# tesseract-robotics/trajopt

Measured on AMD Instinct MI355X. Metric: SQP iters/s (+ QP solves/s), 7-DOF x 30-wp x 1024-batch glass_upright, higher is better.
Workload: dtype f64; 1 GPU; config 1: glass_upright 7-DOF 30-waypoint, collision cost, batch=1024 random seeds per GPU; n_dof=7, n_steps=30, batch_per_gpu=1024, qp_n=572, qp_m=876, parallelism=seeds sharded, dp1

## Files before the change

trajopt_amd/csrc/tmx_api.cpp:

```cpp
#include <algorithm>
#include <cstddef>
#include <limits>
#include <string>
#include <vector>

#include "tmx_kernels.h"
#include "tmx_wave_kernels.h"
#include "tmx_wave_plan.h"
#include "tmx_row_perm.h"
#include "tmx_upload.h"

#ifdef TMX_HOST_EMU
#include <chrono>
thread_local tmx_emu_idx tmx_emu_threadIdx, tmx_emu_blockIdx, tmx_emu_blockDim, tmx_emu_gridDim;
thread_local double* tmx_emu_smem = nullptr;
double tmx_emu_now_ms()
{
  return std::chrono::duration<double, std::milli>(std::chrono::steady_clock::now().time_since_epoch()).count();
}
#else
#include <rccl/rccl.h>
#endif

#define HIPCHK(call)                                                                                                  \
// ... 1396 lines not shown
    int acc = 0, rows_max = 0, naux_max = 0;
    for (int t = 0; t <= T; ++t)
    {
      pl.pst[t] = acc;
      if (t == T)
        break;
      const int c = L.wp_start[t + 1] - L.wp_start[t];
      for (int u = L.wp_start[t]; u < L.wp_start[t + 1]; ++u)
        pl.epos[L.wp_list[u]] = acc + (u - L.wp_start[t]);
      acc += c + (c & 1);
      rows_max = std::max(rows_max, c);
    }
    for (int r = 0; r < R; ++r)
      naux_max = std::max(naux_max, L.naux[r]);
    pl.setup_fast = (rows_max <= TMX_SETUP_COL && naux_max <= 2 && R <= 2 * TMX_QP_NT) ? 1 : 0;
    pl.polish_fast = 0;
    if (pl.setup_fast && dpart_fits(D, T) && R2 == 0)
    {
      DPart dp;
      dpart_make(T, dp);
      const size_t gn = (size_t)dp.Lmax * D, g_doubles = (size_t)dp.P * gn * dpart_gstride((int)gn);
      pl.polish_fast = polish_fast_doubles(T, D * T, R, NA, acc + TMX_SETUP_COL) <= g_doubles ? 1 : 0;
    }
  }
  pl.smem_small = small_smem_bytes(L, P);
#if TMX_IS_DEVICE
  {
    std::vector<int> plan(TMX_WV_NT * TMX_WV_REC, 0);
    int gmax = 4, aux2 = 0, n3 = 0;
    if (hooks.wave == '1' && P.flavor == 0 && R2 == 0 && pl.coef_far == 0 && !E.qp_dense && !P.st && !P.band && !P.use_time && P.n_fx == 0 &&
        wave_plan_build(D, T, R, L.st.data(), L.naux.data(), plan.data(), &gmax, &aux2, &n3))
    {
      const size_t lds = std::max(pl.smem_small, wave_lds_doubles(D, T, R) * sizeof(double));
      if (lds <= 40 * 1024)
      {
        pl.plan.swap(plan);
        pl.wave_ok = 1;
        pl.wv_gmax = gmax;
        pl.wv_aux2 = aux2;
        pl.smem_wave = lds;
      }
    }
  }
#endif
  pl.smem_qp = qp_smem_bytes(D, T, R, NA, R2, pl.coef_far);
  if (P.tt_chain > 0 || P.tv_chain)
// ... 97 lines not shown
  UP(cp_target, L.cp_target);
  UP(ls_link, L.ls_link);
  UP(ls_center, L.ls_center);
  UP(ls_radius, L.ls_radius);
  UP(ob_center, L.ob_center);
  UP(ob_radius, L.ob_radius);
  UP(ob_axis, L.ob_axis);
  UP(tv_owner, L.tv_owner);
  UP(tv_joint, L.tv_joint);
  UP(tv_first, L.tv_first);
  UP(tv_last, L.tv_last);
  UP(tv_coeff, L.tv_coeff);
  UP(tv_target, L.tv_target);
  UP(tv_up, L.tv_up);
  UP(tv_lo, L.tv_lo);
  UP(tt_owner, L.tt_owner);
  UP(tt_form, L.tt_form);
  UP(tt_slot, L.tt_slot);
  UP(tt_coeff, L.tt_coeff);
  UP(tt_limit, L.tt_limit);
  P.coef_far = pl.coef_far;
  P.setup_fast = pl.setup_fast;
  P.polish_fast = pl.polish_fast;
  P.tt_place = pl.tt_place;
  P.wave_ok = pl.wave_ok;
  P.wv_gmax = pl.wv_gmax;
  P.wv_aux2 = pl.wv_aux2;
  if (!pl.row_perm.empty())
    UP(row_perm, pl.row_perm);
  UP(wp_pst, pl.pst);
  UP(row_epos, pl.epos);
  if (pl.wave_ok)
    UP(wv_plan, pl.plan);
#undef UP
  if (!ctx->dp)
  {
    void* p = nullptr;
    HIPCHK(hipMalloc(&p, sizeof(DevProblem)));
    ctx->dp = static_cast<DevProblem*>(p);
  }
  HIPCHK(hipMemcpy(ctx->dp, &P, sizeof(DevProblem), hipMemcpyHostToDevice));
  return TMX_OK;
}

static tmx_status configure_launch(tmx_ctx* ctx, const DevProblem& P, const Lowered& L, const EngineChoice& E, const Placement& pl, const UploadHooks& hooks)
{
// ... 1465 lines not shown
  if (!ctx || !ctx->have_problem || !ctx->dp)
    return TMX_ERR_INVALID;
  TMX_REFUSE_WHILE_PENDING(ctx);
  HIPCHK(hipSetDevice(ctx->device));
  ctx->hp.dbg_flags = flags;
  HIPCHK(hipMemcpy(reinterpret_cast<char*>(ctx->dp) + offsetof(DevProblem, dbg_flags), &flags, sizeof(int), hipMemcpyHostToDevice));
  return TMX_OK;
}

__attribute__((visibility("default"))) int tmx_debug_setup_fast(tmx_ctx* ctx)
{
  if (!ctx || !ctx->have_problem)
    return -1;
  return ctx->hp.setup_fast;
}

__attribute__((visibility("default"))) int tmx_debug_polish_fast(tmx_ctx* ctx)
{
  if (!ctx || !ctx->have_problem)
    return -1;
  return ctx->hp.polish_fast;
}

__attribute__((visibility("default"))) tmx_status tmx_debug_set_fused(tmx_ctx* ctx, int mode)
{
  if (!ctx || mode < 0 || mode > 2)
    return TMX_ERR_INVALID;
  ctx->mode = mode;
  return TMX_OK;
}

tmx_status tmx_kernel_stats_reset(tmx_ctx* ctx)
{
  if (!ctx)
    return TMX_ERR_INVALID;
  ctx->ms_admm = ctx->ms_convexify = ctx->ms_evaluate = 0.0;
  ctx->launches_admm = 0;
  return TMX_OK;
}
}
```

trajopt_amd/csrc/tmx_kernels.h:

```cpp
#pragma once
#include "tmx_solve.h"
#include "tmx_generic.h"

#define TMX_WORK(smem, Bt) ((Bt)->ws_hbm ? (Bt)->ws_hbm + (size_t)blockIdx.x * (size_t)(Bt)->ws_hbm_stride : (smem))

template <bool HULL>
TMX_DEVFN void prepare_body(const DevProblem* P, const DevBatch* Bt)
{
  TMX_SMEM(smem);
  const int b = blockIdx.x, tid = threadIdx.x, NT = blockDim.x;
  const int NX = P->NX, D = P->D, R = P->R;
  const double* x0 = Bt->x0 + (size_t)b * NX;
  double* x = Bt->x + (size_t)b * NX;
  for (int v = tid; v < NX; v += NT)
  {
    const int j = v % D;
    double y = fmax(P->jl[j] + 1e-6, x0[v]);
    y = fmin(P->ju[j] - 1e-6, x0[v]);
    x[v] = (P->flavor == 1) ? x0[v] : y;
  }
  int* act = Bt->active + (size_t)b * R;
  for (int r = tid; r < R; r += NT)
    act[r] = 0;
  for (int k = tid; k < P->n_cnts; k += NT)
// ... 356 lines not shown
#ifdef TMX_PROFILE
  long long tp0 = TMX_CLK();
  const long long wall0 = wall_clock64();
#endif
  if (P->sqp.max_time < 1e300)
  {
    if (tid == 0)
      sqp_time_limit_check(P, Bt, b);
    TMX_SYNC();
    if (Bt->phase[b] == PHASE_DONE)
      return;
  }
  if (Bt->phase[b] == PHASE_CONVEXIFY)
  {
    convexify_terms(P, x, act, coef, Bt->coef2 + (size_t)b * P->n_link * D, rhs, smem, tid, NT, Bt->rowc + (size_t)b * R, Bt->qdyn + (size_t)b * NX);
#ifdef TMX_PROFILE
    if (tid == 0)
    {
      const long long tnow = TMX_CLK();
      Bt->prof[(size_t)b * 16 + 4] += tnow - tp0;
      tp0 = tnow;
    }
#endif
    QpWs cwd;
    qp_structure(P, act, coef, Bt->coef2 + (size_t)b * P->n_link * D, rhs, x, Bt->trust[b], Bt->merit + (size_t)b * P->n_cnts, Bt->dims + 4 * b,
                 Bt->hashes + 4 * b, nullptr, reinterpret_cast<int*>(smem), tid, NT, Bt->qdyn + (size_t)b * NX, compact_lists_of(cwd, P, Bt, b));
#if TMX_LINK_ROWS
    if (P->flavor == 1)
      sqp2_begin_qp(P, Bt, b, smem, tid, NT);
#endif
  }
  TMX_SYNC();
#ifdef TMX_PROFILE
  if (tid == 0)
    Bt->prof[(size_t)b * 16 + 11] += TMX_CLK() - tp0;
#endif
  qp_solve_block<HBM, BANDK, false>(P, Bt, b, smem, tid, NT, chain_lds);
#ifdef TMX_PROFILE
  tp0 = TMX_CLK();
#endif
  for (int v = tid; v < NX; v += NT)
    xn[v] = xq[v];
  TMX_SYNC();
  evaluate_terms(P, xn, Bt->new_cost_vals + (size_t)b * P->n_costs, Bt->new_cnt_viols + (size_t)b * P->n_cnts, smem, tid, NT);
#if TMX_LINK_ROWS
  if (P->flavor == 1)
    sqp2_update_block(P, Bt, b, smem, tid, NT);
  else
#endif
    sqp_update_block(P, Bt, b, smem, tid, NT);
  TMX_SYNC();
#ifdef TMX_PROFILE
  if (tid == 0)
  {
    Bt->prof[(size_t)b * 16 + 12] += TMX_CLK() - tp0;
    Bt->prof[(size_t)b * 16 + 1] += wall_clock64() - wall0;
  }
#endif
}

TMX_KERNEL_LB2(TMX_QP_NT, TMX_QP_WGS_PER_CU) k_sqp_fused(const DevProblem* P, const DevBatch* Bt, int max_steps)
{
  TMX_SMEM(smem);
  const int b = blockIdx.x, tid = threadIdx.x, NT = blockDim.x;
  for (int step = 0; max_steps == 0 || step < max_steps; ++step)
  {
    if (Bt->phase[b] == PHASE_DONE)
      break;
    if (P->band)
      sqp_step_block<false, true>(P, Bt, b, smem, tid, NT);
    else
      sqp_step_block<false, false>(P, Bt, b, smem, tid, NT);
  }
// ... 297 lines not shown
```

trajopt_amd/csrc/tmx_setup.h:

```cpp
#pragma once
#include "tmx_qp.h"

#if TMX_IS_DEVICE
struct SetupRow
{
  int r, t, na, ao, epos;
  bool on;
  double c[8], sa[2], bba[2], qa[2], Da[2], Eba[2], Er;
};

TMX_DEVFN double ruiz_fast(const QpWs& w, const DevProblem* P, int n_pass, int n, int tid)
{
  constexpr int NT = TMX_QP_NT;
  const int D = w.D, T = w.T, NX = w.NX, R = w.R;
  for (int e = tid; e < T * 8; e += NT)
    w.tp[e] = 0.0;
  for (int e = tid; e < R + T + TMX_SETUP_COL; e += NT)
    w.hr[e] = 0.0;
  SetupRow g[2];
  {
    const int* rperm = P->row_perm;
#pragma unroll
    for (int q = 0; q < 2; ++q)
    {
      SetupRow& s = g[q];
      const int slot = q * NT + tid;
// ... 202 lines not shown
```

trajopt_amd/csrc/tmx_solve.h:

```cpp
#pragma once
#include "tmx_qp.h"
#include "tmx_setup.h"
#include "tmx_polish.h"
#include "tmx_terms.h"

#if TMX_IS_DEVICE
#define TMX_ATOMIC_ADD_U64(ptr, v) atomicAdd((unsigned long long*)(ptr), (unsigned long long)(v))
#else
#define TMX_ATOMIC_ADD_U64(ptr, v) __atomic_fetch_add((unsigned long long*)(ptr), (unsigned long long)(v), __ATOMIC_RELAXED)
#endif

TMX_DEVFN double aux_cost(const DevProblem* P, const double* merit, int r)
{
  if (P->flavor == 1)
  {
    const double cf = (P->slot_kind[r] == SLOT_COLLISION_LVS) ? P->slot_objc[r] : P->slot_scale[r];
    return (P->slot_iscnt[r] ? merit[P->slot_owner[r]] : 1.0) * cf;
  }
  return P->slot_iscnt[r] ? merit[P->slot_owner[r]] : P->slot_objc[r];
}
TMX_DEVFN double primary_q(const DevProblem* P, const double* qdyn, int v)
{
  if (P->flavor == 1)
    return (fabs(qdyn[v]) < 1e-7) ? 0.0 : qdyn[v];
  return P->pq[v];
}

TMX_DEVFN double aux_sign(int naux, int k) { return (naux == 1) ? -1.0 : (k == 0 ? 1.0 : -1.0); }

struct CscOut
{
  long long *P_p, *P_i, *A_p, *A_i;
// ... 53 lines not shown
      {
        const int sgm = side ? t - 1 : t;
        if (sgm < P->tv_first[c] || sgm >= P->tv_last[c])
          continue;
        const double* rec = tv_aff + ((size_t)c * P->T + sgm) * TMX_TV_REC;
        double cf = 0.0;
        if (j == P->D - 1)
          cf = side ? rec[2] : 0.0;
        else if (j == P->tv_joint[c])
          cf = side ? rec[1] : rec[0];
        if (half)
          cf = -cf;
        const double lin = ((2 * rec[3 + half]) * cf) * P->tv_coeff[c];
        if (lin != 0.0)
          qv += lin;
      }
  return qv;
}

template <bool ST = false>
TMX_DEVFN void qp_structure(const DevProblem* P, const int* active, const double* coef, const double* coef2, const double* rhs,
                            const double* xcur, double trust, const double* merit, int* dims, unsigned long long* hashes,
                            const CscOut* out, int* iscratch, int tid, int NT, const double* qdyn = nullptr, QpWs* cw = nullptr,
                            const double* fxH = nullptr, const double* fxg = nullptr, const double* tv_aff = nullptr, const double* tt_aff = nullptr)
{
  (void)coef2;
  (void)fxH;
  (void)fxg;
  (void)tv_aff;
  (void)tt_aff;
  const int D = P->D, T = P->T, NX = P->NX, R = P->R;
  int* colptr = iscratch;
  int* rowref = colptr + P->n_max + 1;
  int* auxref = rowref + R;
  int* lact = auxref + R;
  int* lnaux = lact + R;
  int* ccount = lnaux + R;
  int acc_off = 2 * (P->n_max + 1) + 4 * R;
  acc_off += (acc_off & 1);
  unsigned long long* acc = reinterpret_cast<unsigned long long*>(iscratch + acc_off);
  int* scan = iscratch + acc_off + 16;
  for (int r = tid; r < R; r += NT)
  {
    lact[r] = active[r] ? 1 : 0;
    lnaux[r] = P->slot_naux[r];
  }
  for (int k = tid; k < 8; k += NT)
// ... 85 lines not shown
    ccount[v] = c;
  }
  for (int rq = tid; rq < n_it; rq += NT)
  {
    const int r = ali ? ali[rq] : rq;
    if (lact[r])
      for (int k = 0; k < lnaux[r]; ++k)
        ccount[auxref[r] + k] = 2;
  }
  TMX_SYNC();
  for (int c = tid; c <= n; c += NT)
  {
    int run = 0;
    for (int q = 0; q < c; ++q)
      run += ccount[q];
    colptr[c] = run;
    if (c == n)
    {
      dims[3] = run;
      dims[2] = P->nnzP;
    }
  }
  TMX_SYNC();
  const int nnzA = dims[3];
  unsigned long long hA = 0ULL, wsA = 0ULL;
  const int cp_bytes = n + 1, cp_full = cp_bytes / 8, cp_rem = cp_bytes % 8;
  const int ri_bytes = nnzA, ri_full = ri_bytes / 8, ri_rem = ri_bytes % 8;
  for (int c = tid; c <= n; c += NT)
  {
    const long long val = colptr[c];
    hA += tmx_hash_term(val, (uint64_t)c, 3);
    if (c < cp_full)
      wsA += tmx_hash_term(val, (uint64_t)c, 13);
    else if (c == cp_full && cp_rem > 0)
      wsA += tmx_hash_term((long long)((unsigned long long)val & ((1ULL << (8 * cp_rem)) - 1ULL)), (uint64_t)c, 13);
  }
  for (int v = tid; v < NX; v += NT)
  {
    const int t = v / D, j = v % D;
    int pos = colptr[v];
#if TMX_LINK_ROWS
    int ql = (P->n_link > 0 && t > 0) ? wls[t - 1] : 0;
    const int ql_end = (P->n_link > 0 && t > 0) ? wls[t] : 0;
    auto link_val = [&](int qq) -> double {
      const int rr = wll[qq];
      return (active[rr] && P->slot_c2[rr] >= 0) ? coef2[P->slot_c2[rr] * D + j] : 0.0;
// ... 141 lines not shown
    const int r = ali ? ali[rq] : rq;
    if (active[r])
      for (int k = 0; k < P->slot_naux[r]; ++k)
      {
        const int col = auxref[r] + k;
        int pos = colptr[col];
        for (int e = 0; e < 2; ++e)
        {
          const long long ri = (e == 0) ? rowref[r] : (mg + col);
          hA += tmx_hash_term(ri, (uint64_t)pos, 4);
          if (pos < ri_full)
            wsA += tmx_hash_term(ri, (uint64_t)pos, 14);
          else if (pos == ri_full && ri_rem > 0)
            wsA += tmx_hash_term((long long)((unsigned long long)ri & ((1ULL << (8 * ri_rem)) - 1ULL)), (uint64_t)pos, 14);
          if (out)
          {
            out->A_i[pos] = ri;
            out->A_x[pos] = (e == 0) ? aux_sign(P->slot_naux[r], k) : 1.0;
          }
          ++pos;
        }
      }
  }
  unsigned long long hP = 0ULL, wsP = 0ULL;
  bool p_done = false;
  if constexpr (ST)
    if ((fxH != nullptr && P->n_fx_cost > 0) || (tv_aff != nullptr && P->n_tv > 0) || (tt_aff != nullptr && P->n_tt > 0))
    {
      p_done = true;
      TMX_SYNC();
      int* pcnt = ccount;
      const int T1 = P->T + 1;
      auto fx_val = [&](int t, int i, int j, bool& any) -> double {
        double v = 0.0;
        any = false;
        if (fxH == nullptr)
          return v;
        for (int c = 0; c < P->n_fx; ++c)
          if (fx_is_quad(P->fx_kind[c]) && P->fx_t[c] == t)
          {
            const double h = fxH[(size_t)P->fx_ci[c] * D * D + i * D + j];
            const double coeff = (i == j) ? h / 2 : h;
            if (coeff != 0.0)
            {
              v += (i == j) ? 2.0 * coeff : coeff;
              any = true;
// ... 1098 lines not shown
      w.row_epos[P->wp_list[u]] = acc + (u - P->wp_start[t]);
  }
#if TMX_LINK_ROWS
  w.c2i = P->slot_c2;
#endif
  w.sigma = st.sigma;
  w.alpha = st.alpha;
  w.c = 1.0;
  w.cinv = 1.0;
  TMX_SYNC();
  {
    int* scan = reinterpret_cast<int*>(w.red);
    const int C = (R + NT - 1) / NT;
    const int r0 = tid * C < R ? tid * C : R, r1 = (tid + 1) * C < R ? (tid + 1) * C : R;
    for (int pass = 0; pass < 2; ++pass)
    {
      int cnt = 0;
      for (int r = r0; r < r1; ++r)
        cnt += w.act[r] ? (pass == 0 ? 1 : w.naux[r]) : 0;
      int off = 0;
#if TMX_IS_DEVICE
      if (fast_setup)
      {
        const int lane = tid & 63, wave = tid >> 6;
        const unsigned long long below = (1ull << lane) - 1ull;
        int tot = 0;
        for (int bit = 0; bit < 3; ++bit)
        {
          const unsigned long long mk = __builtin_amdgcn_ballot_w64(((cnt >> bit) & 1) != 0);
          off += __builtin_popcountll(mk & below) << bit;
          tot += __builtin_popcountll(mk) << bit;
        }
        TMX_SYNC();
        if (lane == 0)
          scan[wave] = tot;
        TMX_SYNC();
        for (int u = 0; u < wave; ++u)
          off += scan[u];
      }
      else
#endif
      {
        TMX_SYNC();
        scan[tid] = cnt;
        TMX_SYNC();
        for (int u = 0; u < tid; ++u)
          off += scan[u];
      }
      for (int r = r0; r < r1; ++r)
      {
        if (pass == 0)
          w.row_ref[r] = off;
        else
          w.aux_ref[r] = NX + off;
        off += w.act[r] ? (pass == 0 ? 1 : w.naux[r]) : 0;
      }
    }
    TMX_SYNC();
    rows_compact_build(w, P, scan, tid, NT);
  }
  const int n = dims[0], m = dims[1], mg = m - n;
// ... 1101 lines not shown
                for (int tt = 1; tt < P->T; ++tt)
                {
                  if (g[tt] == 0.0)
                    continue;
                  val += (((g[tt] * g[tt]) * w) * xq[tt * D + D - 1]) * xq[tt * D + D - 1];
                  for (int t2 = tt + 1; t2 < P->T; ++t2)
                    if (g[t2] != 0.0)
                      val += (((2 * g[tt] * g[t2]) * w) * xq[tt * D + D - 1]) * xq[t2 * D + D - 1];
                }
                acc += val;
              }
          }
        model_cost[k] = acc;
      }
      else
        model_viol[k - P->n_costs] = acc;
    }
    TMX_SYNC();
  }
}

TMX_DEVFN void sqp_decide(const DevProblem* P, const DevBatch* Bt, int b, const double* model_cost, const double* model_viol);
template <bool ST = false>
TMX_DEVFN void sqp_update_block(const DevProblem* P, const DevBatch* Bt, int b, double* smem, int tid, int NT)
{
  const int NX = P->NX;
  double* model_cost = smem;
  double* model_viol = model_cost + P->n_costs;
  double* cost_vals = Bt->cost_vals + (size_t)b * P->n_costs;
  double* cnt_viols = Bt->cnt_viols + (size_t)b * P->n_cnts;
  const double* new_cost = Bt->new_cost_vals + (size_t)b * P->n_costs;
  const double* new_viol = Bt->new_cnt_viols + (size_t)b * P->n_cnts;
  const bool solved = Bt->cvx[b] == TMX_CVX_SOLVED && Bt->phase[b] != PHASE_DONE;
  if (solved)
    sqp_model_values<ST>(P, Bt, b, Bt->xq + (size_t)b * P->n_max, smem, tid, NT);
  if (tid == 0)
  {
    Bt->accept_flag[b] = 0;
    sqp_decide(P, Bt, b, model_cost, model_viol);
  }
  TMX_SYNC();
  if (Bt->accept_flag[b])
  {
    double* x = Bt->x + (size_t)b * NX;
    const double* xn = Bt->xnew + (size_t)b * NX;
    for (int v = tid; v < NX; v += NT)
      x[v] = xn[v];
    for (int k = tid; k < P->n_costs; k += NT)
      cost_vals[k] = new_cost[k];
    for (int k = tid; k < P->n_cnts; k += NT)
      cnt_viols[k] = new_viol[k];
  }
}

TMX_DEVFN void sqp_decide(const DevProblem* P, const DevBatch* Bt, int b, const double* model_cost, const double* model_viol)
{
  const tmx_sqp_params& sp = P->sqp;
  const double* cost_vals = Bt->cost_vals + (size_t)b * P->n_costs;
  const double* cnt_viols = Bt->cnt_viols + (size_t)b * P->n_cnts;
  const double* new_cost = Bt->new_cost_vals + (size_t)b * P->n_costs;
  const double* new_viol = Bt->new_cnt_viols + (size_t)b * P->n_cnts;
  double* merit = Bt->merit + (size_t)b * P->n_cnts;
  const double* cur_cost = cost_vals;
  const double* cur_viol = cnt_viols;
  int phase = Bt->phase[b];
  if (phase == PHASE_DONE)
    return;
  enum
  {
    GO_WHILE,
    GO_AFTER_WHILE,
    GO_PENALTY,
    GO_CLEANUP
  } next;
  int retval = Bt->retval[b];
  double box = Bt->trust[b];
  Bt->n_qp[b] += 1;
  if (Bt->cvx[b] != TMX_CVX_SOLVED)
  {
    step_log_write(P, Bt, b, 0, box, nullptr, nullptr, nullptr, nullptr, nullptr, nullptr, nullptr, 0.0, 0.0, 0.0, 0.0, 0.0, 0.0);
    if (Bt->qp_fail[b] < sp.max_qp_solver_failures - 1)
    {
      box *= sp.trust_shrink_ratio;
      Bt->qp_fail[b] += 1;
      next = GO_WHILE;
    }
    else if (Bt->qp_fail[b] == sp.max_qp_solver_failures - 1)
    {
      box = sp.min_trust_box_size;
      Bt->qp_fail[b] += 1;
      next = GO_WHILE;
    }
    else
    {
      retval = TMX_OPT_FAILED;
      next = GO_CLEANUP;
    }
  }
  else
  {
    double old_merit = 0.0, model_merit = 0.0, new_merit = 0.0;
    for (int k = 0; k < P->n_costs; ++k)
    {
      old_merit += cost_vals[k];
      model_merit += model_cost[k];
      new_merit += new_cost[k];
    }
    double d0 = 0.0, d1 = 0.0, d2 = 0.0;
    for (int k = 0; k < P->n_cnts; ++k)
    {
      d0 += cnt_viols[k] * merit[k];
      d1 += model_viol[k] * merit[k];
      d2 += new_viol[k] * merit[k];
    }
    old_merit += d0;
    model_merit += d1;
    new_merit += d2;
    const double approx = old_merit - model_merit;
    const double exact = old_merit - new_merit;
    const double ratio = exact / approx;
    Bt->n_fe[b] += 1;
    step_log_write(P, Bt, b, 1, box, cost_vals, model_cost, new_cost, cnt_viols, model_viol, new_viol, merit, old_merit, model_merit, new_merit,
                   approx, exact, ratio);
    if (approx < sp.min_approx_improve)
    {
      retval = TMX_OPT_CONVERGED;
      next = GO_PENALTY;
    }
    else if (approx / old_merit < sp.min_approx_improve_frac)
    {
      retval = TMX_OPT_CONVERGED;
      next = GO_PENALTY;
    }
    else if (exact < 0 || ratio < sp.improve_ratio_threshold)
    {
      box *= sp.trust_shrink_ratio;
      next = GO_WHILE;
    }
    else
    {
      Bt->accept_flag[b] = 1;
      cur_cost = new_cost;
      cur_viol = new_viol;
      box *= sp.trust_expand_ratio;
      next = GO_AFTER_WHILE;
    }
// ... 25 lines not shown
      retval = viol_ok ? TMX_OPT_CONVERGED : TMX_OPT_SCO_ITERATION_LIMIT;
      next = GO_CLEANUP;
    }
    else
    {
      Bt->iter[b] += 1;
      Bt->qp_fail[b] = 0;
      Bt->trust[b] = box;
      Bt->phase[b] = PHASE_CONVEXIFY;
      Bt->retval[b] = retval;
      return;
    }
  }
  if (next == GO_PENALTY)
  {
    if (viol_ok)
      next = GO_CLEANUP;
    else
    {
      if (sp.inflate_constraints_individually)
      {
        for (int k = 0; k < P->n_cnts; ++k)
          if (cur_viol[k] > sp.cnt_tolerance)
            merit[k] *= sp.merit_coeff_increase_ratio;
      }
      else
        for (int k = 0; k < P->n_cnts; ++k)
          merit[k] *= sp.merit_coeff_increase_ratio;
      box = fmax(box, sp.min_trust_box_size / sp.trust_shrink_ratio * 1.5);
      Bt->merit_inc[b] += 1;
      if ((double)Bt->merit_inc[b] < sp.max_merit_coeff_increases)
      {
        Bt->iter[b] = 1;
        Bt->qp_fail[b] = 0;
        Bt->trust[b] = box;
        Bt->phase[b] = PHASE_CONVEXIFY;
        Bt->retval[b] = retval;
        return;
      }
      retval = TMX_OPT_PENALTY_ITERATION_LIMIT;
      next = GO_CLEANUP;
    }
  }
  Bt->trust[b] = box;
  Bt->status[b] = retval;
  Bt->retval[b] = retval;
  double tot = 0.0;
  for (int k = 0; k < P->n_costs; ++k)
    tot += cur_cost[k];
  Bt->total_cost[b] = tot;
  Bt->phase[b] = PHASE_DONE;
// ... 356 lines not shown
```

trajopt_amd/csrc/tmx_types.h:

```cpp
#pragma once
#include "../../include/tmx.h"
#include "tmx_platform.h"

enum
{
  SLOT_FIXED = 0,
  SLOT_CARTPOSE = 1,
  SLOT_JOINTPOS = 2,
  SLOT_COLLISION = 3,
  SLOT_JOINTPOS_INEQ = 4,
  SLOT_JOINTVEL = 5,
  SLOT_JOINTVEL_INEQ = 6,
  SLOT_COLLISION_LVS = 7,
  SLOT_FUNC = 9,
  SLOT_CARTVEL = 8,
  SLOT_JOINTVEL_TIME = 10,
  SLOT_TOTAL_TIME = 11
};
#ifndef TMX_LINK_ROWS
#define TMX_LINK_ROWS 1
#endif

enum
{
// ... 56 lines not shown
  int band_rows;
  int* ls_hull;
  double* hull;
  int n_ls_hull;
  int DK;
  int use_time;
  int n_tv;
  int *tv_owner, *tv_joint, *tv_first, *tv_last;
  double *tv_coeff, *tv_target, *tv_up, *tv_lo;
  int n_tt;
  int *tt_owner, *tt_form, *tt_slot;
  double *tt_coeff, *tt_limit;
  int wave_ok;
  int wv_gmax;
  int wv_aux2;
  int* wv_plan;
  int* row_perm;
  int dbg_flags;
  int tt_chain, tt_place;
  int tv_chain;
  int *wp_pst, *row_epos;
  int setup_fast;
  int polish_fast;
};
TMX_HOSTDEVFN int slot_is_diff(int kind) { return kind == SLOT_JOINTVEL || kind == SLOT_JOINTVEL_INEQ; }
#define TMX_TV_REC 5
TMX_HOSTDEVFN int fx_is_quad(int kind) { return kind == 0 || kind == 1 || kind == 3; }
TMX_HOSTDEVFN int fx_is_rows(int kind) { return kind == 2 || kind == 4; }

struct DevBatch
{
  int B, max_rec;
  double *x0, *x, *xnew;
  double *cost_vals, *cnt_viols, *new_cost_vals, *new_cnt_viols, *merit;
  double *trust, *total_cost, *prev_rho;
  int *phase, *iter, *merit_inc, *qp_fail, *status, *retval, *n_fe, *n_qp, *cvx, *prev_ok;
  int *active;
  double *coef, *rhs;
  double *qdyn;
  double *rowc;
  int *solver_init;
  double *coef2;
  int *dims;
  unsigned long long *hashes;
  int *prev_dims;
  unsigned long long *prev_ws;
// ... 42 lines not shown
```

trajopt_amd/csrc/tmx_upload.h:

```cpp
#pragma once
#include <cstddef>
#include <cstdlib>
#include <string>
#include <vector>

struct Lowered
{
  std::vector<int> kind, st, sub, sub2, owner, naux, iscnt, iseq;
  std::vector<double> objc, scale, aux1, aux2;
  std::vector<int> c2, sub3;
  std::vector<double> aux3;
  std::vector<int> aoff;
  std::vector<double> pd, po, pq, po2, po3;
  std::vector<int> p_colptr;
  std::vector<int> fx_t, fx_kind, fx_owner, fx_op0, fx_nops, fx_c0, fx_nout, fx_slot0, fx_ci, fx_ops;
  std::vector<double> fx_consts;
  std::vector<int> vel_first, vel_last, vel_cost, vel_kind, cp_t, cp_owner, cp_iscnt, cp_nrows, cp_idx, cp_slot0;
  std::vector<double> vel_coeffs, vel_targets, cp_coeff, cp_target;
  std::vector<int> tv_owner, tv_joint, tv_first, tv_last, tt_owner, tt_form, tt_slot;
  std::vector<double> tv_coeff, tv_target, tv_up, tv_lo, tt_coeff, tt_limit;
  std::vector<int> ls_link, ls_hull;
  std::vector<double> ls_center, ls_radius, ob_center, ob_radius, ob_axis, ls_axis, ob_box, hullv, mesh;
  std::vector<int> wp_start, wp_list;
  int R = 0, R2 = 0, NA = 0;
// ... 28 lines not shown
  static UploadHooks read()
  {
    auto first = [](const char* name) {
      const char* e = std::getenv(name);
      return e ? e[0] : '\0';
    };
    UploadHooks h;
    h.total_time_chain = first("TMX_TOTAL_TIME_CHAIN");
    h.vel_time_chain = first("TMX_VEL_TIME_CHAIN");
    h.force_coef_far = first("TMX_FORCE_COEF_FAR");
    h.force_compact = first("TMX_FORCE_COMPACT");
    h.row_perm = first("TMX_ROW_PERM");
    h.wave = first("TMX_WAVE");
    h.tt_place = first("TMX_TT_PLACE");
    const char* e = std::getenv("TMX_DENSE_QP_MAX_N");
    h.dense_qp_max_n = e ? std::max(1, std::atoi(e)) : 448;
    h.verbose = std::getenv("TMX_VERBOSE") != nullptr;
    return h;
  }
};

struct Placement
{
  int coef_far = 0, setup_fast = 0, polish_fast = 0, tt_place = 0;
  int wave_ok = 0, wv_gmax = 2, wv_aux2 = 0;
  std::vector<int> row_perm, pst, epos, plan;
  size_t smem_qp = 0, smem_small = 0, smem_wave = 0;
  size_t tt_scratch = 0;
};
```

Before: 164,000 SQP iters/s.

## Add specialized fast paths for QP structure build and SQP step update

Adds a specialized qp_structure_fast that computes the QP sparsity column pointers and structure hashes with wave-ballot and shuffle prefix scans over per-thread variables. It also adds sqp_update_fast, which stages cost, violation and merit arrays in LDS before the single-thread accept/reject decision and then writes the step log cooperatively. Both run as noinline outlined functions, gated by a host-computed step_fast flag. The aim is to cut serial and global-memory-heavy work in the per-iteration setup and update phases, at the cost of more code paths and added eligibility conditions.

```diff
diff --git a/trajopt_amd/csrc/tmx_api.cpp b/trajopt_amd/csrc/tmx_api.cpp
--- a/trajopt_amd/csrc/tmx_api.cpp
+++ b/trajopt_amd/csrc/tmx_api.cpp
@@ -1442,6 +1442,12 @@
       const size_t gn = (size_t)dp.Lmax * D, g_doubles = (size_t)dp.P * gn * dpart_gstride((int)gn);
       pl.polish_fast = polish_fast_doubles(T, D * T, R, NA, acc + TMX_SETUP_COL) <= g_doubles ? 1 : 0;
     }
+    const size_t eval_room = tmx_eval_scratch_doubles(R, D * T, (int)L.vel_first.size(), L.n_costs, L.n_cnts);
+    pl.step_fast = (pl.setup_fast && dpart_fits(D, T) && R >= 1 && 2 * (size_t)L.n_costs + 3 * (size_t)L.n_cnts + TMX_STEP_LOG_HEAD + 1 <= eval_room && R2 == 0 && D * T <= TMX_QP_NT && P.n_max + 1 <= TMX_STEP_CP_PASSES * TMX_QP_NT && P.flavor == 0 &&
+                    !P.st && !P.band && !P.band_rows && !E.qp_dense && !P.use_time && P.n_fx == 0 && P.n_stencil == 0 && P.n_tt == 0 && P.n_tv == 0 &&
+                    !(pl.coef_far & 2))
+                       ? 1
+                       : 0;
   }
   pl.smem_small = small_smem_bytes(L, P);
 #if TMX_IS_DEVICE
@@ -1585,6 +1591,7 @@
   P.coef_far = pl.coef_far;
   P.setup_fast = pl.setup_fast;
   P.polish_fast = pl.polish_fast;
+  P.step_fast = pl.step_fast;
   P.tt_place = pl.tt_place;
   P.wave_ok = pl.wave_ok;
   P.wv_gmax = pl.wv_gmax;
@@ -3096,6 +3103,13 @@
   return ctx->hp.polish_fast;
 }
 
+__attribute__((visibility("default"))) int tmx_debug_step_fast(tmx_ctx* ctx)
+{
+  if (!ctx || !ctx->have_problem)
+    return -1;
+  return ctx->hp.step_fast;
+}
+
 __attribute__((visibility("default"))) tmx_status tmx_debug_set_fused(tmx_ctx* ctx, int mode)
 {
   if (!ctx || mode < 0 || mode > 2)
diff --git a/trajopt_amd/csrc/tmx_kernels.h b/trajopt_amd/csrc/tmx_kernels.h
--- a/trajopt_amd/csrc/tmx_kernels.h
+++ b/trajopt_amd/csrc/tmx_kernels.h
@@ -1,5 +1,6 @@
 #pragma once
 #include "tmx_solve.h"
+#include "tmx_step.h"
 #include "tmx_generic.h"
 
 #define TMX_WORK(smem, Bt) ((Bt)->ws_hbm ? (Bt)->ws_hbm + (size_t)blockIdx.x * (size_t)(Bt)->ws_hbm_stride : (smem))
@@ -402,9 +403,25 @@
       tp0 = tnow;
     }
 #endif
-    QpWs cwd;
-    qp_structure(P, act, coef, Bt->coef2 + (size_t)b * P->n_link * D, rhs, x, Bt->trust[b], Bt->merit + (size_t)b * P->n_cnts, Bt->dims + 4 * b,
-                 Bt->hashes + 4 * b, nullptr, reinterpret_cast<int*>(smem), tid, NT, Bt->qdyn + (size_t)b * NX, compact_lists_of(cwd, P, Bt, b));
+#if TMX_IS_DEVICE
+    if (TMX_UNI_B(!HBM && NT == TMX_QP_NT && P->step_fast != 0 && !(P->dbg_flags & 8) && TMX_FAST_ALLOWED))
+    {
+#if TMX_ADMM_OUTLINED && TMX_STEP_OUTLINED && !(defined(TMX_PROFILE) && defined(TMX_FINE))
+      unsigned lds_off = (unsigned)(size_t)smem;
+      TMX_ASM_OPAQUE_SGPR(lds_off);
+      qp_structure_fast_nl(P, Bt, b, lds_off);
+#else
+      qp_structure_fast(P, act, coef, Bt->dims + 4 * b, Bt->hashes + 4 * b, reinterpret_cast<int*>(smem), tid TMX_F5_ARGS(&tp0, Bt->prof + (size_t)b * 16));
+#endif
+    }
+    else
+#endif
+    {
+      QpWs cwd;
+      qp_structure(P, act, coef, Bt->coef2 + (size_t)b * P->n_link * D, rhs, x, Bt->trust[b], Bt->merit + (size_t)b * P->n_cnts, Bt->dims + 4 * b,
+                   Bt->hashes + 4 * b, nullptr, reinterpret_cast<int*>(smem), tid, NT, Bt->qdyn + (size_t)b * NX, compact_lists_of(cwd, P, Bt, b),
+                   nullptr, nullptr, nullptr, nullptr TMX_F5_ARGS(&tp0, Bt->prof + (size_t)b * 16));
+    }
 #if TMX_LINK_ROWS
     if (P->flavor == 1)
       sqp2_begin_qp(P, Bt, b, smem, tid, NT);
@@ -423,12 +440,30 @@
     xn[v] = xq[v];
   TMX_SYNC();
   evaluate_terms(P, xn, Bt->new_cost_vals + (size_t)b * P->n_costs, Bt->new_cnt_viols + (size_t)b * P->n_cnts, smem, tid, NT);
+#if defined(TMX_PROFILE) && defined(TMX_FINE) && TMX_FINE == 5
+  [[maybe_unused]] long long* const f5_tl = &tp0;
+  [[maybe_unused]] long long* const f5_pc = Bt->prof + (size_t)b * 16;
+#endif
+  TMX_F5_TICK(13);
+#if TMX_IS_DEVICE
+  if (TMX_UNI_B(!HBM && NT == TMX_QP_NT && P->step_fast != 0 && !(P->dbg_flags & 8) && TMX_FAST_ALLOWED))
+  {
+#if TMX_ADMM_OUTLINED && TMX_STEP_OUTLINED && !(defined(TMX_PROFILE) && defined(TMX_FINE))
+    unsigned lds_off = (unsigned)(size_t)smem;
+    TMX_ASM_OPAQUE_SGPR(lds_off);
+    sqp_update_fast_nl(P, Bt, b, lds_off);
+#else
+    sqp_update_fast(P, Bt, b, smem, tid TMX_F5_ARGS(&tp0, Bt->prof + (size_t)b * 16));
+#endif
+  }
+  else
+#endif
 #if TMX_LINK_ROWS
   if (P->flavor == 1)
     sqp2_update_block(P, Bt, b, smem, tid, NT);
   else
 #endif
-    sqp_update_block(P, Bt, b, smem, tid, NT);
+    sqp_update_block(P, Bt, b, smem, tid, NT TMX_F5_ARGS(&tp0, Bt->prof + (size_t)b * 16));
   TMX_SYNC();
 #ifdef TMX_PROFILE
   if (tid == 0)
diff --git a/trajopt_amd/csrc/tmx_setup.h b/trajopt_amd/csrc/tmx_setup.h
--- a/trajopt_amd/csrc/tmx_setup.h
+++ b/trajopt_amd/csrc/tmx_setup.h
@@ -2,6 +2,26 @@
 #include "tmx_qp.h"
 
 #if TMX_IS_DEVICE
+TMX_DEVFN int block_excl_count8(int cnt, int* scan, int tid)
+{
+  const int lane = tid & 63, wave = tid >> 6;
+  const unsigned long long below = (1ull << lane) - 1ull;
+  int off = 0, tot = 0;
+  for (int bit = 0; bit < 3; ++bit)
+  {
+    const unsigned long long mk = __builtin_amdgcn_ballot_w64(((cnt >> bit) & 1) != 0);
+    off += __builtin_popcountll(mk & below) << bit;
+    tot += __builtin_popcountll(mk) << bit;
+  }
+  TMX_SYNC();
+  if (lane == 0)
+    scan[wave] = tot;
+  TMX_SYNC();
+  for (int u = 0; u < wave; ++u)
+    off += scan[u];
+  return off;
+}
+
 struct SetupRow
 {
   int r, t, na, ao, epos;
diff --git a/trajopt_amd/csrc/tmx_solve.h b/trajopt_amd/csrc/tmx_solve.h
--- a/trajopt_amd/csrc/tmx_solve.h
+++ b/trajopt_amd/csrc/tmx_solve.h
@@ -8,6 +8,25 @@
 #define TMX_ATOMIC_ADD_U64(ptr, v) atomicAdd((unsigned long long*)(ptr), (unsigned long long)(v))
 #else
 #define TMX_ATOMIC_ADD_U64(ptr, v) __atomic_fetch_add((unsigned long long*)(ptr), (unsigned long long)(v), __ATOMIC_RELAXED)
+#endif
+
+#if defined(TMX_PROFILE) && defined(TMX_FINE) && TMX_FINE == 5
+#define TMX_F5_PARAMS , long long *f5_tl = nullptr, long long *f5_pc = nullptr
+#define TMX_F5_ARGS(tl, pc) , (tl), (pc)
+#define TMX_F5_TICK(slot)                                                                                             \
+  do                                                                                                                  \
+  {                                                                                                                   \
+    if (tid == 0 && f5_pc != nullptr)                                                                                 \
+    {                                                                                                                 \
+      const long long now_ = TMX_CLK();                                                                               \
+      f5_pc[slot] += now_ - *f5_tl;                                                                                   \
+      *f5_tl = now_;                                                                                                  \
+    }                                                                                                                 \
+  } while (0)
+#else
+#define TMX_F5_PARAMS
+#define TMX_F5_ARGS(tl, pc)
+#define TMX_F5_TICK(slot) ((void)0)
 #endif
 
 TMX_DEVFN double aux_cost(const DevProblem* P, const double* merit, int r)
@@ -107,7 +126,7 @@
 TMX_DEVFN void qp_structure(const DevProblem* P, const int* active, const double* coef, const double* coef2, const double* rhs,
                             const double* xcur, double trust, const double* merit, int* dims, unsigned long long* hashes,
                             const CscOut* out, int* iscratch, int tid, int NT, const double* qdyn = nullptr, QpWs* cw = nullptr,
-                            const double* fxH = nullptr, const double* fxg = nullptr, const double* tv_aff = nullptr, const double* tt_aff = nullptr)
+                            const double* fxH = nullptr, const double* fxg = nullptr, const double* tv_aff = nullptr, const double* tt_aff = nullptr TMX_F5_PARAMS)
 {
   (void)coef2;
   (void)fxH;
@@ -239,6 +258,7 @@
     }
   }
   TMX_SYNC();
+  TMX_F5_TICK(15);
   const int nnzA = dims[3];
   unsigned long long hA = 0ULL, wsA = 0ULL;
   const int cp_bytes = n + 1, cp_full = cp_bytes / 8, cp_rem = cp_bytes % 8;
@@ -426,6 +446,7 @@
         }
       }
   }
+  TMX_F5_TICK(6);
   unsigned long long hP = 0ULL, wsP = 0ULL;
   bool p_done = false;
   if constexpr (ST)
@@ -1570,21 +1591,7 @@
 #if TMX_IS_DEVICE
       if (fast_setup)
       {
-        const int lane = tid & 63, wave = tid >> 6;
-        const unsigned long long below = (1ull << lane) - 1ull;
-        int tot = 0;
-        for (int bit = 0; bit < 3; ++bit)
-        {
-          const unsigned long long mk = __builtin_amdgcn_ballot_w64(((cnt >> bit) & 1) != 0);
-          off += __builtin_popcountll(mk & below) << bit;
-          tot += __builtin_popcountll(mk) << bit;
-        }
-        TMX_SYNC();
-        if (lane == 0)
-          scan[wave] = tot;
-        TMX_SYNC();
-        for (int u = 0; u < wave; ++u)
-          off += scan[u];
+        off = block_excl_count8(cnt, scan, tid);
       }
       else
 #endif
@@ -2732,7 +2739,7 @@
 
 TMX_DEVFN void sqp_decide(const DevProblem* P, const DevBatch* Bt, int b, const double* model_cost, const double* model_viol);
 template <bool ST = false>
-TMX_DEVFN void sqp_update_block(const DevProblem* P, const DevBatch* Bt, int b, double* smem, int tid, int NT)
+TMX_DEVFN void sqp_update_block(const DevProblem* P, const DevBatch* Bt, int b, double* smem, int tid, int NT TMX_F5_PARAMS)
 {
   const int NX = P->NX;
   double* model_cost = smem;
@@ -2744,6 +2751,7 @@
   const bool solved = Bt->cvx[b] == TMX_CVX_SOLVED && Bt->phase[b] != PHASE_DONE;
   if (solved)
     sqp_model_values<ST>(P, Bt, b, Bt->xq + (size_t)b * P->n_max, smem, tid, NT);
+  TMX_F5_TICK(14);
   if (tid == 0)
   {
     Bt->accept_flag[b] = 0;
@@ -2763,14 +2771,41 @@
   }
 }
 
+struct DecideIo
+{
+  const double *cost_vals, *cnt_viols, *new_cost, *new_viol, *merit;
+  double* head;
+};
+TMX_DEVFN void sqp_decide_io(const DevProblem* P, const DevBatch* Bt, int b, const double* model_cost, const double* model_viol, const DecideIo& io);
 TMX_DEVFN void sqp_decide(const DevProblem* P, const DevBatch* Bt, int b, const double* model_cost, const double* model_viol)
 {
+  const DecideIo io = { Bt->cost_vals + (size_t)b * P->n_costs,     Bt->cnt_viols + (size_t)b * P->n_cnts, Bt->new_cost_vals + (size_t)b * P->n_costs,
+                        Bt->new_cnt_viols + (size_t)b * P->n_cnts, Bt->merit + (size_t)b * P->n_cnts,     nullptr };
+  sqp_decide_io(P, Bt, b, model_cost, model_viol, io);
+}
+TMX_DEVFN void sqp_decide_io(const DevProblem* P, const DevBatch* Bt, int b, const double* model_cost, const double* model_viol, const DecideIo& io)
+{
   const tmx_sqp_params& sp = P->sqp;
-  const double* cost_vals = Bt->cost_vals + (size_t)b * P->n_costs;
-  const double* cnt_viols = Bt->cnt_viols + (size_t)b * P->n_cnts;
-  const double* new_cost = Bt->new_cost_vals + (size_t)b * P->n_costs;
-  const double* new_viol = Bt->new_cnt_viols + (size_t)b * P->n_cnts;
+  const double* cost_vals = io.cost_vals;
+  const double* cnt_viols = io.cnt_viols;
+  const double* new_cost = io.new_cost;
+  const double* new_viol = io.new_viol;
+  const double* merit_rd = io.merit;
   double* merit = Bt->merit + (size_t)b * P->n_cnts;
+  auto log_head = [&](int valid, double box_, double old_merit, double model_merit, double new_merit, double approx, double exact, double ratio) {
+    double* h = io.head;
+    h[0] = (double)Bt->merit_inc[b];
+    h[1] = (double)Bt->iter[b];
+    h[2] = box_;
+    h[3] = old_merit;
+    h[4] = model_merit;
+    h[5] = new_merit;
+    h[6] = approx;
+    h[7] = exact;
+    h[8] = ratio;
+    h[9] = (double)valid;
+    h[TMX_STEP_LOG_HEAD] = valid ? 2.0 : 1.0;
+  };
   const double* cur_cost = cost_vals;
   const double* cur_viol = cnt_viols;
   int phase = Bt->phase[b];
@@ -2788,7 +2823,10 @@
   Bt->n_qp[b] += 1;
   if (Bt->cvx[b] != TMX_CVX_SOLVED)
   {
-    step_log_write(P, Bt, b, 0, box, nullptr, nullptr, nullptr, nullptr, nullptr, nullptr, nullptr, 0.0, 0.0, 0.0, 0.0, 0.0, 0.0);
+    if (io.head != nullptr)
+      log_head(0, box, 0.0, 0.0, 0.0, 0.0, 0.0, 0.0);
+    else
+      step_log_write(P, Bt, b, 0, box, nullptr, nullptr, nullptr, nullptr, nullptr, nullptr, nullptr, 0.0, 0.0, 0.0, 0.0, 0.0, 0.0);
     if (Bt->qp_fail[b] < sp.max_qp_solver_failures - 1)
     {
       box *= sp.trust_shrink_ratio;
@@ -2819,9 +2857,9 @@
     double d0 = 0.0, d1 = 0.0, d2 = 0.0;
     for (int k = 0; k < P->n_cnts; ++k)
     {
-      d0 += cnt_viols[k] * merit[k];
-      d1 += model_viol[k] * merit[k];
-      d2 += new_viol[k] * merit[k];
+      d0 += cnt_viols[k] * merit_rd[k];
+      d1 += model_viol[k] * merit_rd[k];
+      d2 += new_viol[k] * merit_rd[k];
     }
     old_merit += d0;
     model_merit += d1;
@@ -2830,8 +2868,11 @@
     const double exact = old_merit - new_merit;
     const double ratio = exact / approx;
     Bt->n_fe[b] += 1;
-    step_log_write(P, Bt, b, 1, box, cost_vals, model_cost, new_cost, cnt_viols, model_viol, new_viol, merit, old_merit, model_merit, new_merit,
-                   approx, exact, ratio);
+    if (io.head != nullptr)
+      log_head(1, box, old_merit, model_merit, new_merit, approx, exact, ratio);
+    else
+      step_log_write(P, Bt, b, 1, box, cost_vals, model_cost, new_cost, cnt_viols, model_viol, new_viol, merit_rd, old_merit, model_merit, new_merit,
+                     approx, exact, ratio);
     if (approx < sp.min_approx_improve)
     {
       retval = TMX_OPT_CONVERGED;
@@ -2903,11 +2944,11 @@
       {
         for (int k = 0; k < P->n_cnts; ++k)
           if (cur_viol[k] > sp.cnt_tolerance)
-            merit[k] *= sp.merit_coeff_increase_ratio;
+            merit[k] = merit_rd[k] * sp.merit_coeff_increase_ratio;
       }
       else
         for (int k = 0; k < P->n_cnts; ++k)
-          merit[k] *= sp.merit_coeff_increase_ratio;
+          merit[k] = merit_rd[k] * sp.merit_coeff_increase_ratio;
       box = fmax(box, sp.min_trust_box_size / sp.trust_shrink_ratio * 1.5);
       Bt->merit_inc[b] += 1;
       if ((double)Bt->merit_inc[b] < sp.max_merit_coeff_increases)
diff --git a/trajopt_amd/csrc/tmx_step.h b/trajopt_amd/csrc/tmx_step.h
--- /dev/null
+++ b/trajopt_amd/csrc/tmx_step.h
@@ -0,0 +1,334 @@
+#pragma once
+#include "tmx_solve.h"
+
+#define TMX_STEP_CP_PASSES 6
+
+#if TMX_IS_DEVICE
+TMX_DEVFN void qp_structure_fast(const DevProblem* P, const int* active, const double* coef, int* dims, unsigned long long* hashes,
+                                 int* iscratch, int tid TMX_F5_PARAMS)
+{
+  constexpr int NT = TMX_QP_NT;
+  const int D = P->D, NX = P->NX, R = P->R;
+  int* colptr = iscratch;
+  int* rowref = colptr + P->n_max + 1;
+  int* auxref = rowref + R;
+  int* lact = auxref + R;
+  int* lnaux = lact + R;
+  int* ccount = lnaux + R;
+  int acc_off = 2 * (P->n_max + 1) + 4 * R;
+  acc_off += (acc_off & 1);
+  unsigned long long* acc = reinterpret_cast<unsigned long long*>(iscratch + acc_off);
+  int* scan = iscratch + acc_off + 16;
+  int* nm = scan + TMX_STEP_CP_PASSES * (NT / 64);
+  for (int r = tid; r < R; r += NT)
+  {
+    lact[r] = active[r] ? 1 : 0;
+    lnaux[r] = P->slot_naux[r];
+  }
+  for (int k = tid; k < 8; k += NT)
+    acc[k] = 0ULL;
+  TMX_SYNC();
+  {
+    const int C = (R + NT - 1) / NT;
+    const int r0 = tid * C < R ? tid * C : R, r1 = (tid + 1) * C < R ? (tid + 1) * C : R;
+    int tot_r = 0;
+    for (int pass = 0; pass < 2; ++pass)
+    {
+      int cnt = 0;
+      for (int r = r0; r < r1; ++r)
+        cnt += lact[r] ? (pass == 0 ? 1 : lnaux[r]) : 0;
+      int off = block_excl_count8(cnt, scan, tid);
+      for (int r = r0; r < r1; ++r)
+      {
+        if (pass == 0)
+          rowref[r] = off;
+        else
+          auxref[r] = NX + off;
+        off += lact[r] ? (pass == 0 ? 1 : lnaux[r]) : 0;
+      }
+      if (tid == NT - 1)
+      {
+        if (pass == 0)
+          tot_r = off;
+        else
+        {
+          dims[0] = NX + off;
+          dims[1] = tot_r + NX + off;
+          nm[0] = NX + off;
+          nm[1] = tot_r + NX + off;
+        }
+      }
+    }
+  }
+  TMX_SYNC();
+  const int n = TMX_UNI_I(nm[0]), m = TMX_UNI_I(nm[1]), mg = m - n;
+  const bool pv = tid < NX;
+  const int v = pv ? tid : 0, vt = v / D, vj = v - vt * D;
+  unsigned mask = 0u;
+  int rref[TMX_SETUP_COL];
+  {
+    const int q0 = P->wp_start[vt], q1 = P->wp_start[vt + 1];
+#pragma unroll
+    for (int k = 0; k < TMX_SETUP_COL; ++k)
+    {
+      const bool ok = pv && q0 + k < q1;
+      const int r = ok ? P->wp_list[q0 + k] : 0;
+      const double cv = ok ? coef[r * D + vj] : 0.0;
+      rref[k] = rowref[r];
+      mask |= (ok && lact[r] != 0 && cv != 0.0) ? (1u << k) : 0u;
+    }
+  }
+  if (pv)
+    ccount[v] = 1 + __builtin_popcount(mask);
+  for (int r = tid; r < R; r += NT)
+    if (lact[r])
+      for (int k = 0; k < lnaux[r]; ++k)
+        ccount[auxref[r] + k] = 2;
+  TMX_SYNC();
+  const int npass = (n + 1 + NT - 1) / NT;
+  const int lane = tid & 63, wave = tid >> 6;
+  int cp[TMX_STEP_CP_PASSES];
+#pragma unroll
+  for (int p = 0; p < TMX_STEP_CP_PASSES; ++p)
+  {
+    cp[p] = 0;
+    if (p < npass)
+    {
+      const int c = p * NT + tid;
+      const int own = c < n ? ccount[c] : 0;
+      int x = own;
+#pragma unroll
+      for (int d = 1; d < 64; d <<= 1)
+      {
+        const int y = __shfl(x, lane >= d ? lane - d : lane, 64);
+        x += lane >= d ? y : 0;
+      }
+      cp[p] = x - own;
+      if (lane == 63)
+        scan[p * (NT / 64) + wave] = x;
+    }
+  }
+  TMX_SYNC();
+  {
+    int base = 0;
+    for (int u = 0; u < wave; ++u)
+      base += scan[u];
+#pragma unroll
+    for (int p = 0; p < TMX_STEP_CP_PASSES; ++p)
+      if (p < npass)
+      {
+        cp[p] += base;
+        const int c = p * NT + tid;
+        if (c <= n)
+          colptr[c] = cp[p];
+        if (c == n)
+        {
+          dims[3] = cp[p];
+          dims[2] = P->nnzP;
+        }
+        if (p + 1 < npass)
+          for (int u = 0; u < NT / 64; ++u)
+            base += scan[p * (NT / 64) + wave + u];
+      }
+  }
+  TMX_SYNC();
+  TMX_F5_TICK(15);
+  const int nnzA = TMX_UNI_I(colptr[n]);
+  unsigned long long hA = 0ULL, wsA = 0ULL;
+  const int cp_bytes = n + 1, cp_full = cp_bytes / 8, cp_rem = cp_bytes % 8;
+  const int ri_bytes = nnzA, ri_full = ri_bytes / 8, ri_rem = ri_bytes % 8;
+#pragma unroll
+  for (int p = 0; p < TMX_STEP_CP_PASSES; ++p)
+  {
+    const int c = p * NT + tid;
+    if (p < npass && c <= n)
+    {
+      const long long val = cp[p];
+      hA += tmx_hash_term(val, (uint64_t)c, 3);
+      if (c < cp_full)
+        wsA += tmx_hash_term(val, (uint64_t)c, 13);
+      else if (c == cp_full && cp_rem > 0)
+        wsA += tmx_hash_term((long long)((unsigned long long)val & ((1ULL << (8 * cp_rem)) - 1ULL)), (uint64_t)c, 13);
+    }
+  }
+  auto row_term = [&](long long ri, int pos) {
+    hA += tmx_hash_term(ri, (uint64_t)pos, 4);
+    if (pos < ri_full)
+      wsA += tmx_hash_term(ri, (uint64_t)pos, 14);
+    else if (pos == ri_full && ri_rem > 0)
+      wsA += tmx_hash_term((long long)((unsigned long long)ri & ((1ULL << (8 * ri_rem)) - 1ULL)), (uint64_t)pos, 14);
+  };
+  if (pv)
+  {
+    int pos = cp[0];
+#pragma unroll
+    for (int k = 0; k < TMX_SETUP_COL; ++k)
+      if (mask & (1u << k))
+      {
+        row_term(rref[k], pos);
+        ++pos;
+      }
+    row_term(mg + v, pos);
+  }
+  for (int r = tid; r < R; r += NT)
+    if (lact[r])
+      for (int k = 0; k < lnaux[r]; ++k)
+      {
+        const int col = auxref[r] + k;
+        const int pos = colptr[col];
+        row_term(rowref[r], pos);
+        row_term(mg + col, pos + 1);
+      }
+  TMX_F5_TICK(6);
+  unsigned long long hP = 0ULL, wsP = 0ULL;
+  {
+    const int pp_bytes = n + 1, pp_full = pp_bytes / 8, pp_rem = pp_bytes % 8;
+    const int pi_full = P->nnzP / 8, pi_rem = P->nnzP % 8;
+    auto p_term = [&](long long row, int run) {
+      hP += tmx_hash_term(row, (uint64_t)run, 2);
+      if (run < pi_full)
+        wsP += tmx_hash_term(row, (uint64_t)run, 12);
+      else if (run == pi_full && pi_rem > 0)
+        wsP += tmx_hash_term((long long)((unsigned long long)row & ((1ULL << (8 * pi_rem)) - 1ULL)), (uint64_t)run, 12);
+    };
+    for (int c = tid; c <= n; c += NT)
+    {
+      int run = (c <= NX) ? P->p_colptr[c] : P->nnzP;
+      const long long val = run;
+      hP += tmx_hash_term(val, (uint64_t)c, 1);
+      if (c < pp_full)
+        wsP += tmx_hash_term(val, (uint64_t)c, 11);
+      else if (c == pp_full && pp_rem > 0)
+        wsP += tmx_hash_term((long long)((unsigned long long)val & ((1ULL << (8 * pp_rem)) - 1ULL)), (uint64_t)c, 11);
+      if (c < NX)
+      {
+        if (c >= D && P->po[c - D] != 0.0)
+        {
+          p_term(c - D, run);
+          ++run;
+        }
+        if (P->pd[c] != 0.0)
+          p_term(c, run);
+      }
+    }
+  }
+  TMX_ATOMIC_ADD_U64(&acc[0], hP);
+  TMX_ATOMIC_ADD_U64(&acc[1], hA);
+  TMX_ATOMIC_ADD_U64(&acc[2], wsP);
+  TMX_ATOMIC_ADD_U64(&acc[3], wsA);
+  TMX_SYNC();
+  if (tid == 0)
+  {
+    hashes[0] = acc[0];
+    hashes[1] = acc[1];
+    hashes[2] = acc[2];
+    hashes[3] = acc[3];
+  }
+  TMX_SYNC();
+}
+
+TMX_DEVFN void sqp_update_fast(const DevProblem* P, const DevBatch* Bt, int b, double* smem, int tid TMX_F5_PARAMS)
+{
+  constexpr int NT = TMX_QP_NT;
+  const int NX = P->NX, nc = P->n_costs, nv = P->n_cnts;
+  double* model_cost = smem;
+  double* model_viol = smem + nc;
+  double* l_cost = model_viol + nv;
+  double* l_new_cost = l_cost + nc;
+  double* l_viol = l_new_cost + nc;
+  double* l_new_viol = l_viol + nv;
+  double* l_merit = l_new_viol + nv;
+  double* head = l_merit + nv;
+  double* cost_vals = Bt->cost_vals + (size_t)b * nc;
+  double* cnt_viols = Bt->cnt_viols + (size_t)b * nv;
+  const double* new_cost = Bt->new_cost_vals + (size_t)b * nc;
+  const double* new_viol = Bt->new_cnt_viols + (size_t)b * nv;
+  const double* merit = Bt->merit + (size_t)b * nv;
+  const bool solved = Bt->cvx[b] == TMX_CVX_SOLVED && Bt->phase[b] != PHASE_DONE;
+  if (solved)
+    sqp_model_values<false>(P, Bt, b, Bt->xq + (size_t)b * P->n_max, smem, tid, NT);
+  TMX_F5_TICK(14);
+  for (int k = tid; k < nc; k += NT)
+  {
+    l_cost[k] = cost_vals[k];
+    l_new_cost[k] = new_cost[k];
+  }
+  for (int k = tid; k < nv; k += NT)
+  {
+    l_viol[k] = cnt_viols[k];
+    l_new_viol[k] = new_viol[k];
+    l_merit[k] = merit[k];
+  }
+  if (tid == 0)
+    head[TMX_STEP_LOG_HEAD] = 0.0;
+  TMX_SYNC();
+  if (tid == 0)
+  {
+    Bt->accept_flag[b] = 0;
+    const DecideIo io = { l_cost, l_viol, l_new_cost, l_new_viol, l_merit, head };
+    sqp_decide_io(P, Bt, b, model_cost, model_viol, io);
+  }
+  TMX_SYNC();
+  const double logged = head[TMX_STEP_LOG_HEAD];
+  if (logged != 0.0)
+  {
+    double* o = Bt->step_log + (size_t)b * Bt->step_log_stride;
+    for (int k = tid; k < 10; k += NT)
+      o[k] = head[k];
+    if (logged == 2.0)
+    {
+      double* q = o + TMX_STEP_LOG_HEAD;
+      for (int k = tid; k < nc; k += NT)
+      {
+        q[k] = l_cost[k];
+        q[nc + k] = model_cost[k];
+        q[2 * nc + k] = l_new_cost[k];
+      }
+      q += 3 * nc;
+      for (int k = tid; k < nv; k += NT)
+      {
+        q[k] = l_viol[k];
+        q[nv + k] = model_viol[k];
+        q[2 * nv + k] = l_new_viol[k];
+        q[3 * nv + k] = l_merit[k];
+      }
+    }
+  }
+  if (Bt->accept_flag[b])
+  {
+    double* x = Bt->x + (size_t)b * NX;
+    const double* xn = Bt->xnew + (size_t)b * NX;
+    for (int v = tid; v < NX; v += NT)
+      x[v] = xn[v];
+    for (int k = tid; k < nc; k += NT)
+      cost_vals[k] = l_new_cost[k];
+    for (int k = tid; k < nv; k += NT)
+      cnt_viols[k] = l_new_viol[k];
+  }
+}
+
+#ifndef TMX_STEP_OUTLINED
+#define TMX_STEP_OUTLINED 1
+#endif
+#if TMX_ADMM_OUTLINED && TMX_STEP_OUTLINED
+__device__ __attribute__((noinline)) static void qp_structure_fast_nl(const DevProblem* P_in, const DevBatch* Bt_in, int b_in, unsigned lds_in)
+{
+  const DevProblem* P = tmx_uniform_ptr(P_in);
+  const DevBatch* Bt = tmx_uniform_ptr(Bt_in);
+  const int b = __builtin_amdgcn_readfirstlane(b_in);
+  const int tid = threadIdx.x;
+  double* smem = (double*)(tmx_lds_d*)(size_t)(unsigned)__builtin_amdgcn_readfirstlane((int)lds_in);
+  qp_structure_fast(P, Bt->active + (size_t)b * P->R, Bt->coef + (size_t)b * P->R * P->D, Bt->dims + 4 * b, Bt->hashes + 4 * b,
+                    reinterpret_cast<int*>(smem), tid);
+}
+__device__ __attribute__((noinline)) static void sqp_update_fast_nl(const DevProblem* P_in, const DevBatch* Bt_in, int b_in, unsigned lds_in)
+{
+  const DevProblem* P = tmx_uniform_ptr(P_in);
+  const DevBatch* Bt = tmx_uniform_ptr(Bt_in);
+  const int b = __builtin_amdgcn_readfirstlane(b_in);
+  const int tid = threadIdx.x;
+  double* smem = (double*)(tmx_lds_d*)(size_t)(unsigned)__builtin_amdgcn_readfirstlane((int)lds_in);
+  sqp_update_fast(P, Bt, b, smem, tid);
+}
+#endif
+#endif
diff --git a/trajopt_amd/csrc/tmx_types.h b/trajopt_amd/csrc/tmx_types.h
--- a/trajopt_amd/csrc/tmx_types.h
+++ b/trajopt_amd/csrc/tmx_types.h
@@ -102,6 +102,7 @@
   int *wp_pst, *row_epos;
   int setup_fast;
   int polish_fast;
+  int step_fast;
 };
 TMX_HOSTDEVFN int slot_is_diff(int kind) { return kind == SLOT_JOINTVEL || kind == SLOT_JOINTVEL_INEQ; }
 #define TMX_TV_REC 5
diff --git a/trajopt_amd/csrc/tmx_upload.h b/trajopt_amd/csrc/tmx_upload.h
--- a/trajopt_amd/csrc/tmx_upload.h
+++ b/trajopt_amd/csrc/tmx_upload.h
@@ -74,7 +74,7 @@
 
 struct Placement
 {
-  int coef_far = 0, setup_fast = 0, polish_fast = 0, tt_place = 0;
+  int coef_far = 0, setup_fast = 0, polish_fast = 0, step_fast = 0, tt_place = 0;
   int wave_ok = 0, wv_gmax = 2, wv_aux2 = 0;
   std::vector<int> row_perm, pst, epos, plan;
   size_t smem_qp = 0, smem_small = 0, smem_wave = 0;
```

Result: faster. 170,200 SQP iters/s (median of 6 runs) (+3.8%).
